# Samirez/Visual_odometry

Measured on AMD Instinct MI355X. Metric: frame-pairs/sec (1280x720, 2000 ORB feats), higher is better.
Workload: dtype u8+f32+f64; 1 GPU; seeded synthetic 1280x720 drone flight (256 distinct rendered views, closed loop), 2000 ORB features/frame, 8 levels = BASELINE config 2; chunk of 257 consecutive frames -> 256 pairs (k, k+1) per GPU per step, each frame detected once; detector=orb, distinct_rendered_frames=256, pair_stride=1, contexts_per_gpu=3, keypoint_order=cv2, poly_solver=fast, matcher=crosscheck, matcher_kernel=mfma_fp4, ransac=5-point, conf 0.99, 1 px, seed 2^64-1, <=1000 iters, parallelism=single GPU, pairs_ok_last_step=256

## Files before the change

### visual_odometry_amd/csrc/cv2order_kernels.hip

```cpp
#include "vo_internal.h"
#include <float.h>

#ifndef CV_THREADS
#define CV_THREADS 256
#endif
#ifndef CV_EPT
#define CV_EPT 4
#endif
#ifndef CV_LDS_CAP
#define CV_LDS_CAP 4096
#endif

__device__ __forceinline__ bool el_gt(uint2 x, uint2 y) { return __uint_as_float(x.x) > __uint_as_float(y.x); }

#define CV_TIE_CAP CV_THREADS
struct Cv2Shared {
    int cnt[2][CV_EPT][CV_THREADS / 64][2];
    int probe[2][CV_THREADS / 64];
    int ntie, nleft;
    uint32_t tie[CV_TIE_CAP], tie_sorted[CV_TIE_CAP], left[CV_TIE_CAP];
    uint8_t is_tie[CV_TIE_CAP];
};

__device__ __forceinline__ void rank2(const bool (&fl)[CV_EPT], const bool (&fr)[CV_EPT], int parity, Cv2Shared& sh,
// ... 265 lines not shown
        for (int j = 0; j < nr; j++) r += sh.tie[j] < p ? 1 : 0;
        sh.tie_sorted[r] = p;
        sh.is_tie[i] = 0;
    }
    __syncthreads();
    for (int i = tid; i < nr; i += CV_THREADS) { const int rel = (int)sh.tie_sorted[i] - first; if (rel < nr) sh.is_tie[rel] = 1; }
    if (tid == 0) sh.nleft = 0;
    __syncthreads();
    {
        const bool fl = tid < nr && first + tid < last && !sh.is_tie[tid];
        const unsigned long long m = __ballot(fl);
        const int lane = tid & 63, wave = tid >> 6;
        if (lane == 0) sh.probe[0][wave] = (int)__popcll(m);
        __syncthreads();
        int before = 0, total = 0;
        for (int w = 0; w < CV_THREADS / 64; w++) { const int c = sh.probe[0][w]; if (w < wave) before += c; total += c; }
        if (fl) sh.left[before + (int)__popcll(m & (lane ? (~0ULL >> (64 - lane)) : 0ULL))] = (uint32_t)(first + tid);
        if (tid == 0) sh.nleft = total;
    }
    __syncthreads();
    const int K = sh.nleft;
    for (int k = tid; k < K; k += CV_THREADS) {
        const int i = (int)sh.left[k], j = (int)sh.tie_sorted[nr - 1 - k];
        const uint2 x = a[i], y = a[j];
        a[i] = y; a[j] = x;
    }
    __syncthreads();
    return first + nr;
}

template <typename PosT>
__device__ int retain_best_cv2(uint2* a, int n, int n_points, PosT* lpos, PosT* rpos, uint2* s_a, uint16_t* s_l, uint16_t* s_r, Cv2Shared& sh)
{
    if (n_points < 0 || n <= n_points) return n;
    if (n_points == 0) return 0;
    const int tid = threadIdx.x;
    int first = 0, last = n;
    const int nth = n_points - 1;
    int depth = 2 * (31 - __clz(n));
    bool done = false;
    introselect_loop(a, first, last, nth, depth, done, CV_LDS_CAP, lpos, rpos, sh);
    if (!done) {
        const int len = last - first;
        for (int i = tid; i < len; i += CV_THREADS) s_a[i] = a[first + i];
        __syncthreads();
        int f2 = 0, l2 = len;
        introselect_loop(s_a, f2, l2, nth - first, depth, done, CV_WAVE_CAP, s_l, s_r, sh);
        if (!done) {
            if (tid < 64) introselect_wave(s_a, f2, l2, nth - first, depth, s_l, s_r);
            __syncthreads();
        }
        for (int i = tid; i < len; i += CV_THREADS) a[first + i] = s_a[i];
        __syncthreads();
    }
    const float ambiguous = __uint_as_float(a[n_points - 1].x);
    const int fast = partition_ge_sparse(a, n_points, n, ambiguous, sh);
    if (fast >= 0) return fast;
    return partition_pass<1>(a, n_points, n, make_uint2(0, 0), ambiguous, lpos, rpos, sh);
}

__global__ __launch_bounds__(CV_THREADS) void k_cv2_order(PyrGeom g, FrameFeat ff, Cv2Buf cb, const int* kept_in)
{
    __shared__ Cv2Shared sh;
    __shared__ uint2 s_a[CV_LDS_CAP];
    __shared__ uint16_t s_l[CV_LDS_CAP], s_r[CV_LDS_CAP];
    const int l = blockIdx.x, f = blockIdx.y, tid = threadIdx.x;
    const LevelGeom lv = g.lv[l];
    const size_t abase = (size_t)f * cb.all_total + cb.all_off[l];
    const uint32_t* all_pos = cb.all_pos + abase;
    const float* all_resp = cb.all_resp + abase;
    uint2* a = cb.work + abase;
    uint32_t* lpos = cb.lpos + abase;
    uint32_t* rpos = cb.rpos + abase;
    const int listed = cb.all_count[f * VO_MAX_LEVELS + l];
    const int n0 = min(listed, cb.all_cap[l]);
    bool bad = listed > cb.all_cap[l];
    for (int i = tid; i < n0; i += CV_THREADS) a[i] = make_uint2(__float_as_uint(all_resp[i]), (uint32_t)i);
    __syncthreads();
    int n = retain_best_cv2(a, n0, g.score_type == 0 ? 2 * lv.quota : lv.quota, lpos, rpos, s_a, s_l, s_r, sh);
    if (g.score_type == 0) {
        const int nc = min(ff.cand_count[f * VO_MAX_LEVELS + l], lv.cand_cap);
        const uint32_t* cpos = ff.cand_pos + (size_t)f * g.cand_total + lv.cand_off;
        const float* cresp = ff.cand_resp + (size_t)f * g.cand_total + lv.cand_off;
        for (int i = tid; i < n; i += CV_THREADS) {
            const uint32_t pos = all_pos[a[i].y];
            int lo = 0, hi = nc;
            while (lo < hi) { const int mid = (lo + hi) >> 1; if (cpos[mid] < pos) lo = mid + 1; else hi = mid; }
            const bool hit = lo < nc && cpos[lo] == pos;
            bad |= !hit;
            a[i].x = __float_as_uint(hit ? cresp[lo] : -FLT_MAX);
        }
        __syncthreads();
        n = retain_best_cv2(a, n, lv.quota, lpos, rpos, s_a, s_l, s_r, sh);
    }
    int out_base = 0;
    for (int k = 0; k < l; k++) out_base += kept_in[f * VO_MAX_LEVELS + k];
    bad |= n != kept_in[f * VO_MAX_LEVELS + l];
    uint32_t* kp_pos = ff.kp_pos + (size_t)f * g.kp_cap;
    int* kp_level = ff.kp_level + (size_t)f * g.kp_cap;
    float* kp_resp = ff.kp_resp + (size_t)f * g.kp_cap;
    const int nw = min(n, kept_in[f * VO_MAX_LEVELS + l]);
    for (int i = tid; i < nw; i += CV_THREADS) {
        const int p = out_base + i;
        if (p < g.kp_cap) { kp_pos[p] = all_pos[a[i].y]; kp_level[p] = l; kp_resp[p] = __uint_as_float(a[i].x); }
    }
    if (bad && tid == 0) atomicOr(&ff.flags[f], 1);
}

void launch_cv2_order(hipStream_t s, const PyrGeom& g, FrameFeat ff, Cv2Buf cb, int F, const int* kept)
{
    hipLaunchKernelGGL(k_cv2_order, dim3(g.nlevels, F), dim3(CV_THREADS), 0, s, g, ff, cb, kept);
}

__global__ __launch_bounds__(CV_THREADS) void k_retain_raw(const float* resp, int n, int n_points, uint2* a, uint32_t* lpos,
                                                          uint32_t* rpos, int* order, int* n_out)
{
    __shared__ Cv2Shared sh;
    __shared__ uint2 s_a[CV_LDS_CAP];
    __shared__ uint16_t s_l[CV_LDS_CAP], s_r[CV_LDS_CAP];
    for (int i = threadIdx.x; i < n; i += CV_THREADS) a[i] = make_uint2(__float_as_uint(resp[i]), (uint32_t)i);
    __syncthreads();
    const int m = retain_best_cv2(a, n, n_points, lpos, rpos, s_a, s_l, s_r, sh);
    for (int i = threadIdx.x; i < m; i += CV_THREADS) order[i] = (int)a[i].y;
    if (threadIdx.x == 0) *n_out = m;
}

void launch_retain_raw(hipStream_t s, const float* resp, int n, int n_points, uint2* a, uint32_t* lpos, uint32_t* rpos,
                       int* order, int* n_out)
{
    hipLaunchKernelGGL(k_retain_raw, dim3(1), dim3(CV_THREADS), 0, s, resp, n, n_points, a, lpos, rpos, order, n_out);
}
```

### visual_odometry_amd/csrc/orb_kernels.hip

```cpp
#include "vo_internal.h"
#include <type_traits>
#include <float.h>
#include <stdlib.h>

__constant__ int8_t c_pattern[256 * 4] = {
#include "orb_pattern.inc"
};
__constant__ int c_umax[16] = {15, 15, 15, 15, 14, 14, 14, 13, 13, 12, 11, 10, 9, 8, 6, 3};
__constant__ int c_gauss7[7] = {18, 34, 49, 55, 49, 34, 18};


typedef short vo_s16x2 __attribute__((ext_vector_type(2)));
typedef unsigned short vo_u16x2 __attribute__((ext_vector_type(2)));
__device__ __forceinline__ uint32_t pk_sub16(uint32_t a, uint32_t b)
{
    return __builtin_bit_cast(uint32_t, __builtin_bit_cast(vo_s16x2, a) - __builtin_bit_cast(vo_s16x2, b));
}
__device__ __forceinline__ uint32_t pk_add16(uint32_t a, uint32_t b)
{
    return __builtin_bit_cast(uint32_t, __builtin_bit_cast(vo_s16x2, a) + __builtin_bit_cast(vo_s16x2, b));
}
__device__ __forceinline__ uint32_t pk_min16(uint32_t a, uint32_t b)
{
    return __builtin_bit_cast(uint32_t, __builtin_elementwise_min(__builtin_bit_cast(vo_s16x2, a), __builtin_bit_cast(vo_s16x2, b)));
// ... 636 lines not shown
            __syncthreads();
            for (int e0 = 0, k = 0; e0 < nc; e0 += 64, k++)
                if ((lose >> k) & 1u) { const int q = s_q[e0 + lane]; s_sc[(q >> 8) * FT_SCW + (q & 255)] = 0; }
            __syncthreads();
        }
    } else {
        for (int i = lane; i < FT_SCH * (FAST_TW + 2); i += 64) {
            const int gr = i / (FAST_TW + 2), cx = 3 + i % (FAST_TW + 2);
            const int gx = x0 - 4 + cx, gy = y0 - 1 + gr;
            if (gx < xlo || gx > xhi || gy < gylo || gy > gyhi) continue;
            s_sc[gr * FT_SCW + cx] = (uint8_t)fast_score_or_zero(s_px + (gr + 3) * FT_PXW + 12 + cx, t);
        }
        __syncthreads();
        uint8_t* s_out = s_px;
        for (int i = lane; i < FAST_TH * FAST_TW; i += 64) {
            const int ty = i / FAST_TW, tx = i % FAST_TW;
            const uint8_t* c = s_sc + (ty + 1) * FT_SCW + 4 + tx;
            const int sv = c[0];
            const bool win = sv && sv > c[-1] && sv > c[1] && sv > c[-FT_SCW - 1] && sv > c[-FT_SCW] && sv > c[-FT_SCW + 1] &&
                             sv > c[FT_SCW - 1] && sv > c[FT_SCW] && sv > c[FT_SCW + 1];
            s_out[i] = win ? (uint8_t)sv : 0;
            const int gx = x0 + tx, gy = y0 + ty;
            const bool keep = win && gx >= g.edge && gx < lv.w - g.edge && gy >= g.edge && gy < lv.h - g.edge;
            if (keep) atomicAdd(&hist[((size_t)f * VO_MAX_LEVELS + l) * 256 + sv], 1u);
            if (!DENSE) {
                const unsigned long long m = __ballot(keep);
                const int slot = nw + (int)__builtin_amdgcn_mbcnt_hi((uint32_t)(m >> 32), __builtin_amdgcn_mbcnt_lo((uint32_t)m, 0u));
                if (keep) my_list[slot] = ((uint32_t)sv << 16) | ((uint32_t)ty << 8) | (uint32_t)tx;
                nw += (int)__popcll(m);
            }
        }
        __syncthreads();
        for (int i = lane; i < FAST_TH * FAST_TW; i += 64) s_sc[(i / FAST_TW + 1) * FT_SCW + 4 + i % FAST_TW] = s_out[i];
        __syncthreads();
    }
    if (!DENSE) {
        FT_STAT(4, nw);
        if (lane == 0) tile_count[(size_t)f * g.ftiles_total + bid] = nw;
        return;
    }
#pragma unroll
    for (int i = lane; i < FAST_TH * (FAST_TW / 16); i += 64) {
        const int ty = i / (FAST_TW / 16), c16 = i % (FAST_TW / 16);
        const int gy = y0 + ty, gx = x0 + 16 * c16;
        const uint32_t* c = (const uint32_t*)(s_sc + (ty + 1) * FT_SCW + 4 + 16 * c16);
        if (gy < lv.h && gx < lv.stride)
            *(uint4*)(score + (size_t)f * g.frame_bytes + lv.off + (size_t)gy * lv.stride + gx) = make_uint4(c[0], c[1], c[2], c[3]);
    }
}

static_assert((FAST_TH * FAST_TW) % 64 == 0, "the dense fallback appends with full-wave ballots");
void launch_fast(hipStream_t s, const uint8_t* pyr, uint8_t* score, uint32_t* hist, const PyrGeom& g, int F,
                 uint32_t* tile_list, int* tile_count)
{
    if (tile_list) { if (g.ftiles_total > 0) hipLaunchKernelGGL(k_fast<false>, dim3(g.ftiles_total, F), dim3(64), 0, s, pyr, score, hist, g, tile_list, tile_count); }
    else hipLaunchKernelGGL(k_fast<true>, dim3(g.dtiles_total, F), dim3(64), 0, s, pyr, score, hist, g, tile_list, tile_count);
}


__device__ __forceinline__ int sel_threshold(const PyrGeom& g, const LevelGeom& lv, const uint32_t* h, int lane)
{
    const int want = g.score_type == 0 ? 2 * lv.quota : lv.quota;
    uint32_t c[4];
    int own = 0;
#pragma unroll
    for (int k = 0; k < 4; k++) { c[k] = h[255 - 4 * lane - k]; own += (int)c[k]; }
    int inc = own;
#pragma unroll
    for (int d = 1; d < 64; d <<= 1) { int v = __shfl_up(inc, d, 64); if (lane >= d) inc += v; }
    int acc = inc - own, T = 0;
#pragma unroll
    for (int k = 0; k < 4; k++) {
        acc += (int)c[k];
        const int score = 255 - 4 * lane - k;
        if (T == 0 && acc >= want && score >= 1) T = score;
    }
    const unsigned long long found = __ballot(T != 0);
    int result = 1;
    if (found) result = __shfl(T, __ffsll((long long)found) - 1, 64);
    if (want <= 0 || lv.w <= 2 * g.edge || lv.h <= 2 * g.edge) result = 256;
    return __builtin_amdgcn_readfirstlane(result);
}

template <bool EMIT, bool ALL>
__device__ __forceinline__ void sel_rows(const uint32_t* tile_list, const int* tile_count, const PyrGeom& g, const FrameFeat& ff,
                                         int* thr, int* chunk_count, const Cv2Buf& cb, uint32_t* s_sel)
{
    const int f = blockIdx.y, lane = threadIdx.x;
    int l = 0;
    while (l + 1 < g.nlevels && (int)blockIdx.x >= g.lv[l + 1].sel_chunk_base) l++;
    const LevelGeom lv = g.lv[l];
    const int chunk = blockIdx.x - lv.sel_chunk_base;
    const int nchunks = (l + 1 < g.nlevels ? g.lv[l + 1].sel_chunk_base : g.sel_chunks_total) - lv.sel_chunk_base;
    const size_t cslot = (size_t)f * g.sel_chunks_total + blockIdx.x;
    const size_t tile0 = (size_t)f * g.ftiles_total + lv.ftile_base + (size_t)chunk * lv.ftiles_x;
    if (!EMIT) {
        const int T = sel_threshold(g, lv, ff.hist + ((size_t)f * VO_MAX_LEVELS + l) * 256, lane);
        int n = 0, na = 0;
        if (ALL || T <= 255)
            for (int t = 0; t < lv.ftiles_x; t++) {
                const int cnt = min(tile_count[tile0 + t], FT_LISTCAP);
                const uint32_t* lst = tile_list + (tile0 + t) * FT_LISTCAP;
                na += cnt;
                for (int j0 = 0; j0 < cnt; j0 += 64) {
                    const int j = j0 + lane;
                    const uint32_t e = j < cnt ? lst[j] : 0u;
                    n += (int)__popcll(__ballot(j < cnt && (int)(e >> 16) >= T));
                }
            }
        if (lane != 0) return;
        chunk_count[cslot] = n;
        if (ALL) cb.chunk_count[cslot] = na;
        if (chunk == 0) thr[f * VO_MAX_LEVELS + l] = T;
        if (blockIdx.x == 0) {
            ff.flags[f] = 0;
            for (int k = 0; k < g.nlevels; k++)
                if ((k + 1 < g.nlevels ? g.lv[k + 1].sel_chunk_base : g.sel_chunks_total) == g.lv[k].sel_chunk_base) {
                    ff.cand_count[f * VO_MAX_LEVELS + k] = 0;
                    if (ALL) cb.all_count[f * VO_MAX_LEVELS + k] = 0;
                }
        }
        return;
    }
    const int T = thr[f * VO_MAX_LEVELS + l];
    if (!ALL && T > 255) {
        if (chunk == 0 && lane == 0) ff.cand_count[f * VO_MAX_LEVELS + l] = 0;
        return;
    }
    int base = 0, abase = 0;
    {
        const size_t c0 = (size_t)f * g.sel_chunks_total + lv.sel_chunk_base;
        for (int c = lane; c < chunk; c += 64) { base += chunk_count[c0 + c]; if (ALL) abase += cb.chunk_count[c0 + c]; }
#pragma unroll
        for (int d = 32; d >= 1; d >>= 1) { base += __shfl_xor(base, d, 64); if (ALL) abase += __shfl_xor(abase, d, 64); }
    }
    const int W32 = (lv.w + 31) >> 5, NW = FAST_TH * W32;
    uint32_t* s_bm = s_sel;
    uint32_t* s_pf = s_sel + NW;
    uint32_t* s_abm = s_sel + 2 * NW;
    uint32_t* s_apf = s_sel + 3 * NW;
    for (int i = lane; i < NW; i += 64) { s_bm[i] = 0u; if (ALL) s_abm[i] = 0u; }
    __syncthreads();
    for (int t = 0; t < lv.ftiles_x; t++) {
        const int cnt = min(tile_count[tile0 + t], FT_LISTCAP);
        const uint32_t* lst = tile_list + (tile0 + t) * FT_LISTCAP;
        for (int j = lane; j < cnt; j += 64) {
            const uint32_t e = lst[j];
            const bool kept = (int)(e >> 16) >= T;
            if (ALL || kept) {
                const uint32_t gx = (uint32_t)(lv.fox + t * FAST_TW) + (e & 255u), wd = ((e >> 8) & 255u) * W32 + (gx >> 5), bit = 1u << (gx & 31u);
                if (ALL) atomicOr(&s_abm[wd], bit);
                if (kept) atomicOr(&s_bm[wd], bit);
            }
        }
    }
    __syncthreads();
    int n, na = 0;
    {
        const int per = (NW + 63) / 64, w0 = lane * per, w1 = min(NW, w0 + per);
        int own = 0, aown = 0;
        for (int wd = w0; wd < w1; wd++) { own += __popc(s_bm[wd]); if (ALL) aown += __popc(s_abm[wd]); }
        int inc = own, ainc = aown;
#pragma unroll
        for (int d = 1; d < 64; d <<= 1) {
            const int v = __shfl_up(inc, d, 64); if (lane >= d) inc += v;
            if (ALL) { const int av = __shfl_up(ainc, d, 64); if (lane >= d) ainc += av; }
        }
        n = __shfl(inc, 63, 64);
        if (ALL) na = __shfl(ainc, 63, 64);
        int acc = inc - own, aacc = ainc - aown;
        for (int wd = w0; wd < w1; wd++) {
            s_pf[wd] = (uint32_t)acc; acc += __popc(s_bm[wd]);
            if (ALL) { s_apf[wd] = (uint32_t)aacc; aacc += __popc(s_abm[wd]); }
        }
    }
    __syncthreads();
    bool overflow = false;
    uint32_t* out_pos = ff.cand_pos + (size_t)f * g.cand_total + lv.cand_off;
    float* out_resp = ff.cand_resp + (size_t)f * g.cand_total + lv.cand_off;
    uint32_t* all_pos = ALL ? cb.all_pos + (size_t)f * cb.all_total + cb.all_off[l] : nullptr;
    float* all_resp = ALL ? cb.all_resp + (size_t)f * cb.all_total + cb.all_off[l] : nullptr;
    const int all_cap = ALL ? cb.all_cap[l] : 0;
    for (int t = 0; t < lv.ftiles_x; t++) {
        const int cnt = min(tile_count[tile0 + t], FT_LISTCAP);
        const uint32_t* lst = tile_list + (tile0 + t) * FT_LISTCAP;
        for (int j = lane; j < cnt; j += 64) {
            const uint32_t e = lst[j];
            const bool kept = (int)(e >> 16) >= T;
            if (ALL || kept) {
                const uint32_t ly = (e >> 8) & 255u, gx = (uint32_t)(lv.fox + t * FAST_TW) + (e & 255u);
                const int wd = (int)(ly * W32 + (gx >> 5));
                const uint32_t below = (1u << (gx & 31u)) - 1u, key = (((uint32_t)(lv.foy + chunk * FAST_TH) + ly) << 16) | gx;
                const float score = (float)(e >> 16);
                if (ALL) {
                    const int apos = abase + (int)s_apf[wd] + __popc(s_abm[wd] & below);
                    if (apos < all_cap) { all_pos[apos] = key; all_resp[apos] = score; }
                    else overflow = true;
                }
                if (kept) {
                    const int pos = base + (int)s_pf[wd] + __popc(s_bm[wd] & below);
                    if (pos < lv.cand_cap) { out_pos[pos] = key; out_resp[pos] = score; }
                    else overflow = true;
                }
            }
        }
    }
    if (overflow) atomicOr(&ff.flags[f], 1);
    if (chunk == nchunks - 1 && lane == 0) {
        ff.cand_count[f * VO_MAX_LEVELS + l] = min(base + n, lv.cand_cap);
        if (ALL) cb.all_count[f * VO_MAX_LEVELS + l] = min(abase + na, all_cap);
    }
}

template <bool EMIT>
__global__ __launch_bounds__(64) void k_sel_rows(const uint32_t* tile_list, const int* tile_count, PyrGeom g, FrameFeat ff,
                                                 int* thr, int* chunk_count)
{
    extern __shared__ uint32_t s_sel[];
    sel_rows<EMIT, false>(tile_list, tile_count, g, ff, thr, chunk_count, Cv2Buf(), s_sel);
}
template <bool EMIT>
__global__ __launch_bounds__(64) void k_sel_rows(const uint32_t* tile_list, const int* tile_count, PyrGeom g, FrameFeat ff,
                                                 int* thr, int* chunk_count, Cv2Buf cb)
{
    extern __shared__ uint32_t s_sel[];
    sel_rows<EMIT, true>(tile_list, tile_count, g, ff, thr, chunk_count, cb, s_sel);
}

static size_t sel_bitmap_bytes(const PyrGeom& g, bool all)
{
    int w = 0;
    for (int l = 0; l < g.nlevels; l++) w = g.lv[l].w > w ? g.lv[l].w : w;
    return (size_t)(all ? 4 : 2) * FAST_TH * ((w + 31) / 32) * 4;
}

void launch_select_fast(hipStream_t s, const PyrGeom& g, FrameFeat ff, int F, int* thr, int* chunk_count,
                        const uint32_t* tile_list, const int* tile_count, const Cv2Buf* cb)
{
    if (g.sel_chunks_total <= 0) {
        (void)hipMemsetAsync(ff.flags, 0, (size_t)F * sizeof(int), s);
        (void)hipMemsetAsync(ff.cand_count, 0, (size_t)F * VO_MAX_LEVELS * sizeof(int), s);
        if (cb) (void)hipMemsetAsync(cb->all_count, 0, (size_t)F * VO_MAX_LEVELS * sizeof(int), s);
        return;
    }
    const dim3 grid(g.sel_chunks_total, F);
    if (cb) {
        hipLaunchKernelGGL(k_sel_rows<false>, grid, dim3(64), 0, s, tile_list, tile_count, g, ff, thr, chunk_count, *cb);
        hipLaunchKernelGGL(k_sel_rows<true>, grid, dim3(64), sel_bitmap_bytes(g, true), s, tile_list, tile_count, g, ff, thr, chunk_count, *cb);
    } else {
        hipLaunchKernelGGL(k_sel_rows<false>, grid, dim3(64), 0, s, tile_list, tile_count, g, ff, thr, chunk_count);
        hipLaunchKernelGGL(k_sel_rows<true>, grid, dim3(64), sel_bitmap_bytes(g, false), s, tile_list, tile_count, g, ff, thr, chunk_count);
    }
}

__global__ __launch_bounds__(256) void k_harris(const uint8_t* pyr, PyrGeom g, FrameFeat ff, int blocks_per_level)
{
    const int bid = xcd_tile(blockIdx.x, gridDim.x);
    const int f = bid / (blocks_per_level * g.nlevels), l = (bid / blocks_per_level) % g.nlevels;
    const int i = (bid % blocks_per_level) * 256 + threadIdx.x;
    const LevelGeom lv = g.lv[l];
    if (i >= min(ff.cand_count[f * VO_MAX_LEVELS + l], lv.cand_cap)) return;
    const size_t ci = (size_t)f * g.cand_total + lv.cand_off + i;
    const uint32_t pos = ff.cand_pos[ci];
    const int x0 = pos & 0xffff, y0 = pos >> 16, st = lv.stride;
    const uint8_t* img = pyr + (size_t)f * g.frame_bytes + lv.off + (size_t)(y0 - 4) * st + (x0 - 4);
    int dxr[9][7], sxr[9][7];
#pragma unroll
    for (int r = 0; r < 9; r++) {
        uint32_t w0, w1, w2;
        __builtin_memcpy(&w0, img + (size_t)r * st, 4);
        __builtin_memcpy(&w1, img + (size_t)r * st + 4, 4);
        __builtin_memcpy(&w2, img + (size_t)r * st + 8, 4);
        int px[9];
#pragma unroll
        for (int c = 0; c < 9; c++) px[c] = (int)(((c < 4 ? w0 : c < 8 ? w1 : w2) >> (8 * (c & 3))) & 255u);
#pragma unroll
        for (int c = 0; c < 7; c++) { dxr[r][c] = px[c + 2] - px[c]; sxr[r][c] = px[c] + 2 * px[c + 1] + px[c + 2]; }
    }
    int a = 0, b = 0, c = 0;
#pragma unroll
    for (int r = 1; r < 8; r++)
#pragma unroll
        for (int k = 0; k < 7; k++) {
            const int Ix = dxr[r - 1][k] + 2 * dxr[r][k] + dxr[r + 1][k];
            const int Iy = sxr[r + 1][k] - sxr[r - 1][k];
            a += Ix * Ix; b += Iy * Iy; c += Ix * Iy;
        }
    const float scale = 1.f / ((1 << 2) * 7 * 255.f);
    const float scale_sq_sq = scale * scale * scale * scale;
    ff.cand_resp[ci] = ((float)a * (float)b - (float)c * (float)c - 0.04f * ((float)a + (float)b) * ((float)a + (float)b)) * scale_sq_sq;
}

void launch_harris(hipStream_t s, const uint8_t* pyr, const PyrGeom& g, FrameFeat ff, int F)
{
    int maxcap = 0;
    for (int l = 0; l < g.nlevels; l++) maxcap = g.lv[l].cand_cap > maxcap ? g.lv[l].cand_cap : maxcap;
    const int bpl = (maxcap + 255) / 256;
    hipLaunchKernelGGL(k_harris, dim3(bpl * g.nlevels * F), dim3(256), 0, s, pyr, g, ff, bpl);
}

__device__ __forceinline__ uint32_t f2key(float v)
{
    uint32_t u = __float_as_uint(v);
    return (u & 0x80000000u) ? ~u : (u | 0x80000000u);
}
__device__ __forceinline__ float key2f(uint32_t k)
{
    return __uint_as_float((k & 0x80000000u) ? (k & 0x7fffffffu) : ~k);
}

__global__ __launch_bounds__(256) void k_harris_threshold(PyrGeom g, FrameFeat ff, float* thr_out, int* kept_out)
{
    __shared__ int s_hist[256];
    __shared__ uint32_t s_prefix;
    __shared__ int s_remaining;
    __shared__ int s_kept;
// ... 563 lines not shown
```

### visual_odometry_amd/csrc/vo_api.hip

```cpp
#include "vo_internal.h"
#include <float.h>
#include <math.h>
#include <stdio.h>
#include <stdlib.h>
#include <string.h>
#include <vector>
#include <type_traits>
#include <algorithm>

#define MAX_EVENTS 384

struct DevList {
    struct Entry { void* p; bool pinned; };
    std::vector<Entry> ptrs;
    DevList() = default;
    DevList(const DevList&) = delete;
    DevList& operator=(DevList&& o) noexcept { if (this != &o) { release(); ptrs.swap(o.ptrs); } return *this; }
    ~DevList() { release(); }
    template <typename T> hipError_t alloc(T** p, size_t n) { return keep(hipMalloc((void**)p, (n ? n : 1) * sizeof(T)), (void**)p, false); }
    template <typename T> hipError_t alloc_pinned(T** p, size_t n)
    {
        return keep(hipHostMalloc((void**)p, (n ? n : 1) * sizeof(T), hipHostMallocDefault), (void**)p, true);
    }
    void release()
// ... 233 lines not shown
        const int iw = lv.w - p->edge_threshold - lv.fox, ih = lv.h - p->edge_threshold - lv.foy;
        const int trows = iw > 0 && ih > 0 ? (ih + FAST_TH - 1) / FAST_TH : 0;
        lv.ftile_base = ft; lv.ftiles_x = trows > 0 ? (iw + FAST_TW - 1) / FAST_TW : 0;
        ft += lv.ftiles_x * trows;
        lv.dtile_base = dt; lv.dtiles_x = (lv.w + FAST_TW - 1) / FAST_TW;
        dt += lv.dtiles_x * ((lv.h + FAST_TH - 1) / FAST_TH);
        lv.btile_base = bt; lv.btiles_x = (lv.w + BLUR_TW - 1) / BLUR_TW;
        bt += lv.btiles_x * ((lv.h + BLUR_TH - 1) / BLUR_TH);
        const int want = p->score_type == 0 ? 2 * lv.quota : lv.quota;
        lv.sel_chunk_base = sc;
        sc += trows;
        lv.cand_off = co;
        lv.cand_cap = align_up(want + (want > 1024 ? want : 1024), 8);
        co += lv.cand_cap;
    }
    g->frame_bytes = align_up(off, 256);
    g->ftiles_total = ft; g->btiles_total = bt; g->dtiles_total = dt;
    g->cand_total = co;
    g->sel_chunks_total = sc;
    g->kp_cap = align_up(p->nfeatures + (p->nfeatures / 8 > 256 ? p->nfeatures / 8 : 256), 8);
    return VO_OK;
}

static void build_lin_tab(int ssize, int dsize, int* ofs, uint16_t* c1, int* pmin, int* pmax)
{
    const double inv_scale = (double)dsize / (double)ssize;
    const double scale = 1.0 / inv_scale;
    int minofst = 0, maxofst = dsize;
    for (int val = 0; val < dsize; val++) {
        volatile double fval = scale * ((double)val + 0.5);
        fval = fval - 0.5;
        const double fv = fval;
        const int ival = cv_floor_d(fv);
        ofs[val] = 0; c1[val] = 0;
        if (ival >= 0 && ssize > 1) {
            if (ival < ssize - 1) {
                ofs[val] = ival;
                volatile double fr = fv - (double)ival;
                fr = fr * 256.0;
                c1[val] = (uint16_t)lrint((double)fr);
            } else {
                ofs[val] = ssize - 1;
                if (val < maxofst) maxofst = val;
            }
        } else if (val + 1 > minofst) minofst = val + 1;
    }
    *pmin = minofst; *pmax = maxofst;
}

static hipError_t alloc_pairbuf(DevList& mem, PairBuf& pb, int P, int cap, bool with_pose_mask)
{
    hipError_t e;
    const size_t pc = (size_t)P * cap;
    pb = PairBuf{};
#define A_(field, n) if ((e = mem.alloc(&pb.field, (n))) != hipSuccess) return e
    A_(slots, (size_t)P * 2); A_(nn_idx, pc * 2); A_(nn_dist, pc * 2); A_(nn_idx2, pc); A_(nn_dist2, pc);
    A_(m_q, pc); A_(m_t, pc); A_(m_d, pc); A_(m_count, (size_t)P);
    A_(px1, pc * 2); A_(px2, pc * 2); A_(xn1, pc * 2); A_(xn2, pc * 2);
    A_(mask, pc); A_(models, (size_t)P * 64 * 90); A_(pose_state, (size_t)P);
    A_(in1, pc * 2); A_(in2, pc * 2); A_(ipx1, pc * 2); A_(ipx2, pc * 2);
    A_(res, (size_t)P); A_(X, pc * 4);
    if (with_pose_mask) { A_(pose_mask, pc); }
    if (const size_t n = nn_colkey_ints(P, cap)) { A_(nn_colkey, n); }
#undef A_
    return hipSuccess;
}

static int alloc_cv2(vo_ctx* ctx)
{
    if (ctx->cv2_ready) return VO_OK;
    const PyrGeom& g = ctx->g;
    Cv2Buf& cb = ctx->cv2;
    int off = 0;
    for (int l = 0; l < g.nlevels; l++) {
        const int px8 = g.lv[l].w * g.lv[l].h / 8 + 1024;
        cb.all_off[l] = off;
        cb.all_cap[l] = align_up(px8 > g.lv[l].cand_cap ? px8 : g.lv[l].cand_cap, 8);
        off += cb.all_cap[l];
    }
    cb.all_total = off;
    const size_t F = (size_t)ctx->max_frames, n = F * off;
    DevList& m = ctx->orb_mem;
    HIPCHK(m.alloc(&cb.all_pos, n)); HIPCHK(m.alloc(&cb.all_resp, n)); HIPCHK(m.alloc(&cb.work, n));
    HIPCHK(m.alloc(&cb.lpos, n)); HIPCHK(m.alloc(&cb.rpos, n));
    HIPCHK(m.alloc(&cb.all_count, F * VO_MAX_LEVELS));
    HIPCHK(m.alloc(&cb.chunk_count, F * (size_t)(g.sel_chunks_total + 1)));
    HIPCHK(hipMemset(cb.all_count, 0, F * VO_MAX_LEVELS * sizeof(int)));
    HIPCHK(hipDeviceSynchronize());
    ctx->cv2_ready = true;
    return VO_OK;
}

static void free_config(vo_ctx* c)
{
    c->configured = c->cv2_ready = false;
    c->orb_mem.release();
    c->pb_mem.release();
    c->pb_pairs = c->pb_cap = 0;
    clear_last_run(c);
}

static void comm_release(vo_ctx* ctx);
static int sift_frames_upload_enqueue(vo_ctx* ctx, const uint8_t* frames, int F, int row_stride, int64_t frame_stride, int first_slot);
static int sift_frames_detect_enqueue(vo_ctx* ctx, int first_slot, int F);

extern "C" int vo_version(void) { return 120; }

extern "C" int vo_create(int device_id, vo_ctx** out)
{
    if (!out) return VO_ERR_INVALID;
    *out = nullptr;
    int ndev = 0;
    if (hipGetDeviceCount(&ndev) != hipSuccess || device_id < 0 || device_id >= ndev) return VO_ERR_HIP;
    vo_ctx* ctx = new vo_ctx();
    ctx->device = device_id;
    if (hipSetDevice(device_id) != hipSuccess || hipStreamCreateWithFlags(&ctx->stream, hipStreamNonBlocking) != hipSuccess ||
        ctx->mem.alloc(&ctx->dK, 16) != hipSuccess) {
        delete ctx;
        return VO_ERR_HIP;
    }
    for (int i = 0; i < MAX_EVENTS; i++) { (void)hipEventCreate(&ctx->ev[i][0]); (void)hipEventCreate(&ctx->ev[i][1]); }
    ctx->ev_ready = true;
    (void)hipEventCreateWithFlags(&ctx->ev_det, hipEventDisableTiming);
    *out = ctx;
    return VO_OK;
}

extern "C" void vo_destroy(vo_ctx* ctx)
{
    if (!ctx) return;
    (void)hipSetDevice(ctx->device);
    (void)hipStreamSynchronize(ctx->stream);
    if (ctx->stream_jpg) { (void)hipStreamSynchronize(ctx->stream_jpg); (void)hipStreamDestroy(ctx->stream_jpg); }
    for (int i = 0; i < 2; i++) if (ctx->ev_jpg[i]) (void)hipEventDestroy(ctx->ev_jpg[i]);
    if (ctx->ev_ready) for (int i = 0; i < MAX_EVENTS; i++) { (void)hipEventDestroy(ctx->ev[i][0]); (void)hipEventDestroy(ctx->ev[i][1]); }
    if (ctx->ev_det) (void)hipEventDestroy(ctx->ev_det);
    comm_release(ctx);
    (void)hipStreamDestroy(ctx->stream);
    delete ctx;
}

enum { NN_POPCOUNT, NN_INT8, NN_FP4 };
static int nn_kernel(const vo_ctx* ctx, int cap)
{
    if (ctx->matcher_kernel == 1 || cap >= 16129) return NN_POPCOUNT;
    return ctx->matcher_kernel == 2 && cap < 8192 ? NN_FP4 : NN_INT8;
}

static int launch_hamming_nn(const vo_ctx* ctx, const PairBuf& pb, const uint8_t* desc, const uint8_t* desc_x, int fp4,
                             const int* kp_count, int cap, int P, int dirs, int knn2)
{
    if (nn_kernel(ctx, cap) == NN_POPCOUNT) { launch_match_nn_popcount(ctx->stream, desc, kp_count, cap, pb, P, dirs, knn2); return 0; }
    return launch_match_nn(ctx->stream, desc_x, kp_count, cap, desc_x_rows(cap), pb, P, dirs, knn2, fp4);
}

extern "C" int vo_set_matcher_kernel(vo_ctx* ctx, int kind)
{
    if (!ctx) return VO_ERR_INVALID;
    if (kind < 0 || kind > 2) FAIL(VO_ERR_INVALID, "matcher kernel must be 0 (int8 MFMA), 1 (XOR + popcount) or 2 (block-scaled FP4 MFMA)");
    ctx->matcher_kernel = kind;
    return VO_OK;
}

extern "C" int vo_set_keypoint_order(vo_ctx* ctx, int kind)
{
    if (!ctx) return VO_ERR_INVALID;
    if (kind != 0 && kind != 1) FAIL(VO_ERR_INVALID, "keypoint order must be 0 (canonical) or 1 (cv2)");
// ... 155 lines not shown
    if (row_stride == ctx->w && frame_stride >= (int64_t)ctx->w * ctx->h) {
        const size_t per = (size_t)ctx->w * ctx->h;
        int rc = ctx->staging.grow(ctx, per * F); if (rc) return rc;
        HIPCHK(hipMemcpy2DAsync(ctx->staging.p, per, frames, (size_t)frame_stride, per, F, hipMemcpyHostToDevice, ctx->stream));
        launch_gray(ctx->stream, ctx->staging.p, 1, ctx->w, (int64_t)per, ctx->pyr + (size_t)first_slot * ctx->g.frame_bytes, ctx->g, F);
        HIPCHK(hipGetLastError());
        return VO_OK;
    }
    for (int f = 0; f < F; f++)
        HIPCHK(hipMemcpy2DAsync(dst0 + (size_t)f * ctx->g.frame_bytes, lv.stride, frames + (size_t)f * frame_stride, row_stride,
                                ctx->w, ctx->h, hipMemcpyHostToDevice, ctx->stream));
    return VO_OK;
}

extern "C" int vo_frames_upload(vo_ctx* ctx, const uint8_t* frames, int F, int row_stride, int64_t frame_stride, int first_slot)
{
    if (!ctx) return VO_ERR_INVALID;
    int rc = frames_upload_enqueue(ctx, frames, F, row_stride, frame_stride, first_slot);
    if (rc) return rc;
    HIPCHK(hipStreamSynchronize(ctx->stream));
    return VO_OK;
}

extern "C" int vo_frames_upload_async(vo_ctx* ctx, const uint8_t* frames, int F, int row_stride, int64_t frame_stride, int first_slot)
{
    if (!ctx) return VO_ERR_INVALID;
    return frames_upload_enqueue(ctx, frames, F, row_stride, frame_stride, first_slot);
}

extern "C" int vo_frames_upload_color(vo_ctx* ctx, const uint8_t* frames, int F, int channels, int row_stride,
                                      int64_t frame_stride, int first_slot)
{
    if (!ctx) return VO_ERR_INVALID;
    if (channels == 1) return vo_frames_upload(ctx, frames, F, row_stride, frame_stride, first_slot);
    const Batch b = batch(ctx);
    if (!b.ready) FAIL(VO_ERR_NOT_CONFIGURED, "vo_batch_configure has not been called");
    if (channels != 3 && channels != 4) FAIL(VO_ERR_INVALID, "channels must be 1, 3 or 4");
    if (!frames || F < 0 || first_slot < 0 || first_slot + F > b.max_frames) FAIL(VO_ERR_INVALID, "slot range out of bounds");
    if (row_stride < b.w * channels || frame_stride < (int64_t)row_stride * b.h) FAIL(VO_ERR_INVALID, "strides too small");
    if (F == 0) return VO_OK;
    HIPCHK(hipSetDevice(ctx->device));
    const size_t per = (size_t)frame_stride;
    const int chunk = F < 64 ? F : 64;
    int rc = ctx->staging.grow(ctx, per * chunk); if (rc) return rc;
    for (int f0 = 0; f0 < F; f0 += chunk) {
        const int n = F - f0 < chunk ? F - f0 : chunk;
        HIPCHK(hipMemcpyAsync(ctx->staging.p, frames + (size_t)f0 * per, per * n, hipMemcpyHostToDevice, ctx->stream));
        StageTimer t(ctx, ST_GRAY);
        gray_into_slots(ctx, ctx->stream, ctx->staging.p, channels, row_stride, frame_stride, first_slot + f0, n);
    }
    HIPCHK(hipGetLastError());
    HIPCHK(hipStreamSynchronize(ctx->stream));
    if (ctx->prof) prof_collect(ctx);
    return VO_OK;
}

static int run_detect(vo_ctx* ctx, int first_slot, int F, int upto)
{
    const PyrGeom& g = ctx->g;
    hipStream_t s = ctx->stream;
    uint8_t* pyr = ctx->pyr + (size_t)first_slot * g.frame_bytes;
    uint8_t* blur = ctx->blur + (size_t)first_slot * g.frame_bytes;
    uint8_t* score = ctx->score + (size_t)first_slot * g.frame_bytes;
    FrameFeat ff = ctx->ff;
    ff.cand_pos += (size_t)first_slot * g.cand_total; ff.cand_resp += (size_t)first_slot * g.cand_total;
    ff.cand_count += (size_t)first_slot * VO_MAX_LEVELS;
    ff.kp_pos += (size_t)first_slot * g.kp_cap; ff.kp_level += (size_t)first_slot * g.kp_cap;
    ff.kp_resp += (size_t)first_slot * g.kp_cap; ff.kp_angle += (size_t)first_slot * g.kp_cap;
    ff.kp_xy += (size_t)first_slot * g.kp_cap * 2; ff.kp_size += (size_t)first_slot * g.kp_cap;
    ff.desc += (size_t)first_slot * g.kp_cap * 32;
    ff.kp_count += first_slot; ff.flags += first_slot;
    ff.hist += (size_t)first_slot * VO_MAX_LEVELS * 256;
    ff.tile_list += (size_t)first_slot * g.ftiles_total * FAST_LISTCAP; ff.tile_count += (size_t)first_slot * g.ftiles_total;
    {
        StageTimer t(ctx, ST_RESIZE);
        for (int l = 1; l < g.nlevels; l++) launch_resize(s, pyr, g, l, ctx->tabs[l], F);
    }
    if (upto < 1) return VO_OK;
    const bool cv2 = ctx->kp_order == 1 && ctx->cv2_ready;
    Cv2Buf cb = ctx->cv2;
    if (cv2) {
        const size_t fo = (size_t)first_slot;
        cb.all_pos += fo * cb.all_total; cb.all_resp += fo * cb.all_total; cb.work += fo * cb.all_total;
        cb.lpos += fo * cb.all_total; cb.rpos += fo * cb.all_total;
        cb.all_count += fo * VO_MAX_LEVELS; cb.chunk_count += fo * g.sel_chunks_total;
    }
    {
        StageTimer t(ctx, ST_MISC);
        HIPCHK(hipMemsetAsync(ff.hist, 0, (size_t)F * VO_MAX_LEVELS * 256 * sizeof(uint32_t), s));
        if (upto < 2) {
            HIPCHK(hipMemsetAsync(ff.flags, 0, (size_t)F * sizeof(int), s));
            HIPCHK(hipMemsetAsync(ff.cand_count, 0, (size_t)F * VO_MAX_LEVELS * sizeof(int), s));
            if (cv2) HIPCHK(hipMemsetAsync(cb.all_count, 0, (size_t)F * VO_MAX_LEVELS * sizeof(int), s));
        }
    }
    { StageTimer t(ctx, ST_FAST); launch_fast(s, pyr, score, ff.hist, g, F, upto < 2 ? nullptr : ff.tile_list, ff.tile_count); }
    if (upto < 2) return VO_OK;
    { StageTimer t(ctx, ST_SELECT_FAST); launch_select_fast(s, g, ff, F, ctx->sel_thr + (size_t)first_slot * VO_MAX_LEVELS, ctx->sel_chunk_count + (size_t)first_slot * g.sel_chunks_total, ff.tile_list, ff.tile_count, cv2 ? &cb : nullptr); }
    if (g.score_type == 0) { StageTimer t(ctx, ST_HARRIS); launch_harris(s, pyr, g, ff, F); }
    { StageTimer t(ctx, ST_SELECT_HARRIS); launch_select_harris(s, g, ff, F, ctx->har_thr + (size_t)first_slot * VO_MAX_LEVELS, ctx->har_kept + (size_t)first_slot * VO_MAX_LEVELS); }
    if (cv2) {
        StageTimer t(ctx, ST_CV2_ORDER);
        launch_cv2_order(s, g, ff, cb, F, ctx->har_kept + (size_t)first_slot * VO_MAX_LEVELS);
    }
    { StageTimer t(ctx, ST_ANGLE); launch_angle(s, pyr, g, ff, F); }
    { StageTimer t(ctx, ST_BLUR); launch_blur(s, pyr, blur, g, F); }
    {
        StageTimer t(ctx, ST_BRIEF);
        const int cx = desc_x_rows(g.kp_cap);
        ctx->descx_fp4 = nn_kernel(ctx, g.kp_cap) == NN_FP4;
        launch_brief(s, blur, g, ff, F, ctx->desc_x + (size_t)first_slot * cx * 256, cx, ctx->descx_fp4);
    }
    return VO_OK;
}

extern "C" int vo_batch_kp_capacity(vo_ctx* ctx)
{
    if (!ctx) return 0;
    const Batch b = batch(ctx);
    return b.ready ? b.kp_cap : 0;
}

extern "C" int vo_host_alloc(size_t bytes, void** out)
{
    if (!out) return VO_ERR_INVALID;
    *out = nullptr;
    return hipHostMalloc(out, bytes ? bytes : 1, hipHostMallocDefault) == hipSuccess ? VO_OK : VO_ERR_HIP;
}

extern "C" void vo_host_free(void* p)
{
    if (p) (void)hipHostFree(p);
}

static int detect_enqueue(vo_ctx* ctx, int first_slot, int F)
{
    const Batch b = batch(ctx);
    if (!b.ready) FAIL(VO_ERR_NOT_CONFIGURED, "vo_batch_configure has not been called");
    if (F < 0 || first_slot < 0 || first_slot + F > b.max_frames) FAIL(VO_ERR_INVALID, "slot range out of bounds");
    HIPCHK(hipSetDevice(ctx->device));
    if (F == 0) return VO_OK;
    if (b.sift) return sift_frames_detect_enqueue(ctx, first_slot, F);
    int rc = run_detect(ctx, first_slot, F, 2);
    if (rc) return rc;
    HIPCHK(hipGetLastError());
    return VO_OK;
}

extern "C" int vo_frames_detect_async(vo_ctx* ctx, int first_slot, int F)
{
    if (!ctx) return VO_ERR_INVALID;
    int rc = detect_enqueue(ctx, first_slot, F);
    if (rc) return rc;
    HIPCHK(hipEventRecord(ctx->ev_det, ctx->stream));
    ctx->ev_det_set = true;
    return VO_OK;
}

extern "C" int vo_detect_after(vo_ctx* ctx, vo_ctx* other)
{
    if (!ctx || !other) return VO_ERR_INVALID;
    if (ctx->device != other->device) FAIL(VO_ERR_INVALID, "the two contexts are on different devices");
    if (ctx == other || !other->ev_det_set) return VO_OK;
    HIPCHK(hipSetDevice(ctx->device));
    HIPCHK(hipStreamWaitEvent(ctx->stream, other->ev_det, 0));
    return VO_OK;
}
// ... 2275 lines not shown
```

### visual_odometry_amd/csrc/vo_internal.h

```cpp
#pragma once
#include <hip/hip_runtime.h>
#include <stdint.h>
#include "../../include/vo_hip.h"

enum {
    ST_GRAY = 0, ST_RESIZE, ST_FAST, ST_SELECT_FAST, ST_HARRIS, ST_SELECT_HARRIS, ST_ANGLE,
    ST_BLUR, ST_BRIEF, ST_MATCH_NN, ST_MATCH_SELECT, ST_RANSAC, ST_POSE, ST_TRIANGULATE,
    ST_MISC, ST_RESERVED, ST_SIFT_SCALE, ST_SIFT_EXTREMA, ST_SIFT_ORIENT, ST_SIFT_SORT, ST_SIFT_DESC, ST_CV2_ORDER, ST_GATHER, ST_RESERVED2,
    ST_SLAM_PREPARE, ST_SLAM_BA, ST_SLAM_FILTER, ST_SLAM_LIMIT
};

struct LevelGeom {
    int w, h, stride, off;
    int quota;
    float scale;
    int ftile_base, ftiles_x;
    int fox, foy;
    int dtile_base, dtiles_x;
    int btile_base, btiles_x;
    int cand_off, cand_cap;
    int sel_chunk_base;
};

struct PyrGeom {
    int nlevels, frame_bytes;
    int edge, fast_thr, score_type, nfeatures;
    int ftiles_total, btiles_total, dtiles_total;
    int cand_total, kp_cap;
    int sel_chunks_total;
    LevelGeom lv[VO_MAX_LEVELS];
};

#define RS2_WW 256
#define RS2_WH 16
#ifndef RS2_WAVES
#define RS2_WAVES 4
#endif
#define RS2_THREADS (64 * RS2_WAVES)
#define RS2_TH (RS2_WAVES * RS2_WH)

struct ResizeTab {
    const int* xofs; const uint16_t* xc1;
    const int* yofs; const uint16_t* yc1;
    int min_x, max_x, min_y, max_y;
    int direct;
};

#ifndef FAST_TW
#define FAST_TW 112
#endif
#ifndef FAST_TH
#define FAST_TH 20
#endif
#define BLUR_TW 128
#ifndef BLUR_TH
#define BLUR_TH 48
#endif
#define FAST_LISTCAP ((FAST_TW / 2) * (FAST_TH / 2))

struct FrameFeat {
    uint32_t* cand_pos;
    float*    cand_resp;
    int*      cand_count;
    uint32_t* kp_pos;
    int*      kp_level;
    float*    kp_resp;
    float*    kp_angle;
    float*    kp_xy;
    float*    kp_size;
    uint8_t*  desc;
    int*      kp_count;
    int*      flags;
    uint32_t* hist;
    uint32_t* tile_list;
    int*      tile_count;
};

struct Cv2Buf {
    uint32_t* all_pos;
    float*    all_resp;
    int*      all_count;
    int*      chunk_count;
    uint2*    work;
    uint32_t* lpos;
    uint32_t* rpos;
    int all_off[VO_MAX_LEVELS], all_cap[VO_MAX_LEVELS], all_total;
};

struct PoseState {
    int active;
    int ninl;
    int good[4];
    double R1[9], R2[9], t[3];
};

struct PairBuf {
    int*      slots;
    int*      nn_idx;
    int*      nn_dist;
    int*      nn_idx2;
    int*      nn_dist2;
    int*      nn_colkey;
    int*      m_q;
    int*      m_t;
    float*    m_d;
    int*      m_count;
    double*   px1;
    double*   px2;
    double*   xn1;
    double*   xn2;
    uint8_t*  mask;
    double*   models;
    PoseState* pose_state;
    double*   in1;
    double*   in2;
    double*   ipx1;
    double*   ipx2;
    vo_pair_result* res;
    double*   X;
    uint8_t*  pose_mask;
};

struct RansacParams {
    double prob, thresh_px;
    int max_iters;
    uint64_t seed;
    double K[9];
    double dist_thresh;
    int dk_early;
};

const char* rccl_load(void);
const char* rccl_unique_id(uint8_t* id128);
const char* rccl_comm_init(void** comm, const uint8_t* id128, int rank, int world);
void rccl_comm_destroy(void* comm);
const char* rccl_comm_count(void* comm, int* n);
const char* rccl_all_gather_f64(void* comm, const double* send, double* recv, size_t count, hipStream_t s);
void launch_pack_records(hipStream_t s, const vo_pair_result* res, int B, int valid, double* rec);

void launch_gray(hipStream_t s, const uint8_t* src, int channels, int row_stride, int64_t frame_stride,
                 uint8_t* pyr, const PyrGeom& g, int F);
void launch_gray_plain(hipStream_t s, const uint8_t* src, int channels, int row_stride, int64_t frame_stride,
                       uint8_t* dst, int w, int h, int dstride, int64_t dframe, int F);
void launch_resize(hipStream_t s, uint8_t* pyr, const PyrGeom& g, int level, const ResizeTab& tab, int F);
void launch_fast(hipStream_t s, const uint8_t* pyr, uint8_t* score, uint32_t* hist, const PyrGeom& g, int F,
                 uint32_t* tile_list, int* tile_count);
void launch_select_fast(hipStream_t s, const PyrGeom& g, FrameFeat ff, int F, int* thr, int* chunk_count,
                        const uint32_t* tile_list, const int* tile_count, const Cv2Buf* cb);
void launch_harris(hipStream_t s, const uint8_t* pyr, const PyrGeom& g, FrameFeat ff, int F);
void launch_cv2_order(hipStream_t s, const PyrGeom& g, FrameFeat ff, Cv2Buf cb, int F, const int* kept);
void launch_retain_raw(hipStream_t s, const float* resp, int n, int n_points, uint2* a, uint32_t* lpos, uint32_t* rpos,
                       int* order, int* n_out);
void launch_select_harris(hipStream_t s, const PyrGeom& g, FrameFeat ff, int F, float* thr, int* kept);
void launch_angle(hipStream_t s, const uint8_t* pyr, const PyrGeom& g, FrameFeat ff, int F);
void launch_resize_linear(hipStream_t st, const uint8_t* src, int sw, int sh, int cn, int sstride, int64_t sframe,
                          uint8_t* dst, int dw, int dh, int dstride, int64_t dframe,
                          const int* xofs, const void* xa, const int* yofs, const void* yb, int area2, int F);
void launch_resize_area(hipStream_t st, const uint8_t* src, int cn, int sstride, uint8_t* dst, int dw, int dh, int dstride,
                        int isx, int isy, const int* xsi, const float* xal, const int* xst, const int* ysi, const float* yal, const int* yst);
#define SIFT_IMG_BORDER 5
#define SIFT_MAX_INTERP_STEPS 5
#define SIFT_MAX_OCT 16
#define SIFT_MAX_TAPS 64
// ... 156 lines not shown
```

Baseline: 98370 frame-pairs/s.

## Flatten FAST tile-list traversal and record candidate indices to skip binary search

The select-FAST kernel now walks the per-tile lists through a wave-wide prefix scan over tile counts, so each lane processes several flattened entries per trip instead of looping tile by tile with mostly idle lanes. The first batch of entries is packed and held in registers across the marking and emit passes. During emit it records each kept entry's candidate index into a new all_cand buffer, which lets the cv2-order kernel replace its per-element binary search over candidate positions with a direct indexed lookup. The prefix arrays can optionally be 16-bit to shrink LDS use. In exchange it adds an extra global buffer and write, more register pressure, and readlane loops over up to 64 tiles per entry batch.

New measurement: 101,000 frame-pairs/s, median of 6. +2.7%, better.

```diff
diff --git a/visual_odometry_amd/csrc/cv2order_kernels.hip b/visual_odometry_amd/csrc/cv2order_kernels.hip
--- a/visual_odometry_amd/csrc/cv2order_kernels.hip
+++ b/visual_odometry_amd/csrc/cv2order_kernels.hip
@@ -371,13 +371,12 @@
         const int nc = min(ff.cand_count[f * VO_MAX_LEVELS + l], lv.cand_cap);
         const uint32_t* cpos = ff.cand_pos + (size_t)f * g.cand_total + lv.cand_off;
         const float* cresp = ff.cand_resp + (size_t)f * g.cand_total + lv.cand_off;
+        const uint32_t* all_cand = cb.all_cand + abase;
         for (int i = tid; i < n; i += CV_THREADS) {
-            const uint32_t pos = all_pos[a[i].y];
-            int lo = 0, hi = nc;
-            while (lo < hi) { const int mid = (lo + hi) >> 1; if (cpos[mid] < pos) lo = mid + 1; else hi = mid; }
-            const bool hit = lo < nc && cpos[lo] == pos;
+            const uint32_t ai = a[i].y, pos = all_pos[ai], idx = all_cand[ai];
+            const bool hit = idx < (uint32_t)nc && cpos[idx] == pos;
             bad |= !hit;
-            a[i].x = __float_as_uint(hit ? cresp[lo] : -FLT_MAX);
+            a[i].x = __float_as_uint(hit ? cresp[idx] : -FLT_MAX);
         }
         __syncthreads();
         n = retain_best_cv2(a, n, lv.quota, lpos, rpos, s_a, s_l, s_r, sh);
diff --git a/visual_odometry_amd/csrc/orb_kernels.hip b/visual_odometry_amd/csrc/orb_kernels.hip
--- a/visual_odometry_amd/csrc/orb_kernels.hip
+++ b/visual_odometry_amd/csrc/orb_kernels.hip
@@ -742,6 +742,43 @@
     return __builtin_amdgcn_readfirstlane(result);
 }
 
+__device__ __forceinline__ int sel_load_counts(const int* tile_count, size_t tile_first, int nt, int lane)
+{
+    return min(tile_count[tile_first + min(lane, max(nt - 1, 0))], FT_LISTCAP);
+}
+__device__ __forceinline__ int sel_scan_counts(int cnt, int nt, int lane, int& total)
+{
+    int inc = cnt;
+#pragma unroll
+    for (int d = 1; d < 64; d <<= 1) { const int v = __shfl_up(inc, d, 64); if (lane >= d) inc += v; }
+    total = __builtin_amdgcn_readlane(inc, max(nt - 1, 0));
+    return inc;
+}
+
+#define SEL_TRIPS 4
+__device__ __forceinline__ void sel_flat_entries(const uint32_t* lists, int nt, int inc, int e, int total,
+                                                 uint32_t (&ent)[SEL_TRIPS], int (&tile)[SEL_TRIPS])
+{
+    int st[SEL_TRIPS];
+#pragma unroll
+    for (int u = 0; u < SEL_TRIPS; u++) { tile[u] = 0; st[u] = 0; }
+    for (int k = 0; k + 1 < nt; k++) {
+        const int v = __builtin_amdgcn_readlane(inc, k);
+#pragma unroll
+        for (int u = 0; u < SEL_TRIPS; u++) if (e + 64 * u >= v) { tile[u] = k + 1; st[u] = v; }
+    }
+#pragma unroll
+    for (int u = 0; u < SEL_TRIPS; u++) ent[u] = lists[e + 64 * u < total ? tile[u] * FT_LISTCAP + (e + 64 * u - st[u]) : 0];
+#pragma unroll
+    for (int u = 0; u < SEL_TRIPS; u++) ent[u] = e + 64 * u < total ? ent[u] : 0u;
+}
+
+#ifdef SEL_PF16
+typedef uint16_t sel_pf_t;
+#else
+typedef uint32_t sel_pf_t;
+#endif
+
 template <bool EMIT, bool ALL>
 __device__ __forceinline__ void sel_rows(const uint32_t* tile_list, const int* tile_count, const PyrGeom& g, const FrameFeat& ff,
                                          int* thr, int* chunk_count, const Cv2Buf& cb, uint32_t* s_sel)
@@ -755,17 +792,22 @@
     const size_t cslot = (size_t)f * g.sel_chunks_total + blockIdx.x;
     const size_t tile0 = (size_t)f * g.ftiles_total + lv.ftile_base + (size_t)chunk * lv.ftiles_x;
     if (!EMIT) {
+        int cnt = sel_load_counts(tile_count, tile0, min(lv.ftiles_x, 64), lane);
         const int T = sel_threshold(g, lv, ff.hist + ((size_t)f * VO_MAX_LEVELS + l) * 256, lane);
         int n = 0, na = 0;
         if (ALL || T <= 255)
-            for (int t = 0; t < lv.ftiles_x; t++) {
-                const int cnt = min(tile_count[tile0 + t], FT_LISTCAP);
-                const uint32_t* lst = tile_list + (tile0 + t) * FT_LISTCAP;
-                na += cnt;
-                for (int j0 = 0; j0 < cnt; j0 += 64) {
-                    const int j = j0 + lane;
-                    const uint32_t e = j < cnt ? lst[j] : 0u;
-                    n += (int)__popcll(__ballot(j < cnt && (int)(e >> 16) >= T));
+            for (int tb = 0; tb < lv.ftiles_x; tb += 64) {
+                const int nt = min(lv.ftiles_x - tb, 64);
+                if (tb) cnt = sel_load_counts(tile_count, tile0 + tb, nt, lane);
+                int total;
+                const int inc = sel_scan_counts(cnt, nt, lane, total);
+                const uint32_t* lists = tile_list + (tile0 + tb) * FT_LISTCAP;
+                na += total;
+                for (int e0 = 0; e0 < total; e0 += 64 * SEL_TRIPS) {
+                    uint32_t ent[SEL_TRIPS]; int tile[SEL_TRIPS];
+                    sel_flat_entries(lists, nt, inc, e0 + lane, total, ent, tile);
+#pragma unroll
+                    for (int u = 0; u < SEL_TRIPS; u++) n += (int)__popcll(__ballot((int)(ent[u] >> 16) >= T));
                 }
             }
         if (lane != 0) return;
@@ -782,6 +824,8 @@
         }
         return;
     }
+    const int nt0 = min(lv.ftiles_x, 64);
+    const int cnt0 = sel_load_counts(tile_count, tile0, nt0, lane);
     const int T = thr[f * VO_MAX_LEVELS + l];
     if (!ALL && T > 255) {
         if (chunk == 0 && lane == 0) ff.cand_count[f * VO_MAX_LEVELS + l] = 0;
@@ -794,26 +838,49 @@
 #pragma unroll
         for (int d = 32; d >= 1; d >>= 1) { base += __shfl_xor(base, d, 64); if (ALL) abase += __shfl_xor(abase, d, 64); }
     }
+    auto pack = [&](uint32_t e, int tile) -> uint32_t {
+        return e ? ((e & 0x00ff0000u) << 8) | ((e & 0x0000ff00u) << 8) | ((uint32_t)(lv.fox + tile * FAST_TW) + (e & 255u)) : 0u;
+    };
+    int total0;
+    const int inc0 = sel_scan_counts(cnt0, nt0, lane, total0);
+    uint32_t held[SEL_TRIPS];
+    {
+        uint32_t ent[SEL_TRIPS]; int tile[SEL_TRIPS];
+        sel_flat_entries(tile_list + tile0 * FT_LISTCAP, nt0, inc0, lane, total0, ent, tile);
+#pragma unroll
+        for (int u = 0; u < SEL_TRIPS; u++) held[u] = pack(ent[u], tile[u]);
+    }
+    auto beyond_held = [&](auto&& visit) {
+        for (int tb = 0; tb < lv.ftiles_x; tb += 64) {
+            const int nt = min(lv.ftiles_x - tb, 64);
+            int total = total0, inc = inc0;
+            if (tb) inc = sel_scan_counts(sel_load_counts(tile_count, tile0 + tb, nt, lane), nt, lane, total);
+            for (int e0 = tb ? 0 : 64 * SEL_TRIPS; e0 < total; e0 += 64 * SEL_TRIPS) {
+                uint32_t ent[SEL_TRIPS]; int tile[SEL_TRIPS];
+                sel_flat_entries(tile_list + (tile0 + tb) * FT_LISTCAP, nt, inc, e0 + lane, total, ent, tile);
+#pragma unroll
+                for (int u = 0; u < SEL_TRIPS; u++) visit(pack(ent[u], tb + tile[u]));
+            }
+        }
+    };
     const int W32 = (lv.w + 31) >> 5, NW = FAST_TH * W32;
     uint32_t* s_bm = s_sel;
-    uint32_t* s_pf = s_sel + NW;
-    uint32_t* s_abm = s_sel + 2 * NW;
-    uint32_t* s_apf = s_sel + 3 * NW;
+    uint32_t* s_abm = s_sel + NW;
+    sel_pf_t* s_pf = (sel_pf_t*)(s_sel + (ALL ? 2 : 1) * NW);
+    sel_pf_t* s_apf = s_pf + NW;
     for (int i = lane; i < NW; i += 64) { s_bm[i] = 0u; if (ALL) s_abm[i] = 0u; }
     __syncthreads();
-    for (int t = 0; t < lv.ftiles_x; t++) {
-        const int cnt = min(tile_count[tile0 + t], FT_LISTCAP);
-        const uint32_t* lst = tile_list + (tile0 + t) * FT_LISTCAP;
-        for (int j = lane; j < cnt; j += 64) {
-            const uint32_t e = lst[j];
-            const bool kept = (int)(e >> 16) >= T;
-            if (ALL || kept) {
-                const uint32_t gx = (uint32_t)(lv.fox + t * FAST_TW) + (e & 255u), wd = ((e >> 8) & 255u) * W32 + (gx >> 5), bit = 1u << (gx & 31u);
-                if (ALL) atomicOr(&s_abm[wd], bit);
-                if (kept) atomicOr(&s_bm[wd], bit);
-            }
-        }
-    }
+    auto mark = [&](uint32_t p) {
+        const bool kept = (int)(p >> 24) >= T;
+        if (ALL ? p != 0u : kept) {
+            const uint32_t gx = p & 0xffffu, wd = ((p >> 16) & 255u) * W32 + (gx >> 5), bit = 1u << (gx & 31u);
+            if (ALL) atomicOr(&s_abm[wd], bit);
+            if (kept) atomicOr(&s_bm[wd], bit);
+        }
+    };
+#pragma unroll
+    for (int u = 0; u < SEL_TRIPS; u++) mark(held[u]);
+    beyond_held(mark);
     __syncthreads();
     int n, na = 0;
     {
@@ -830,8 +897,8 @@
         if (ALL) na = __shfl(ainc, 63, 64);
         int acc = inc - own, aacc = ainc - aown;
         for (int wd = w0; wd < w1; wd++) {
-            s_pf[wd] = (uint32_t)acc; acc += __popc(s_bm[wd]);
-            if (ALL) { s_apf[wd] = (uint32_t)aacc; aacc += __popc(s_abm[wd]); }
+            s_pf[wd] = (sel_pf_t)acc; acc += __popc(s_bm[wd]);
+            if (ALL) { s_apf[wd] = (sel_pf_t)aacc; aacc += __popc(s_abm[wd]); }
         }
     }
     __syncthreads();
@@ -840,31 +907,34 @@
     float* out_resp = ff.cand_resp + (size_t)f * g.cand_total + lv.cand_off;
     uint32_t* all_pos = ALL ? cb.all_pos + (size_t)f * cb.all_total + cb.all_off[l] : nullptr;
     float* all_resp = ALL ? cb.all_resp + (size_t)f * cb.all_total + cb.all_off[l] : nullptr;
+    uint32_t* all_cand = ALL ? cb.all_cand + (size_t)f * cb.all_total + cb.all_off[l] : nullptr;
     const int all_cap = ALL ? cb.all_cap[l] : 0;
-    for (int t = 0; t < lv.ftiles_x; t++) {
-        const int cnt = min(tile_count[tile0 + t], FT_LISTCAP);
-        const uint32_t* lst = tile_list + (tile0 + t) * FT_LISTCAP;
-        for (int j = lane; j < cnt; j += 64) {
-            const uint32_t e = lst[j];
-            const bool kept = (int)(e >> 16) >= T;
-            if (ALL || kept) {
-                const uint32_t ly = (e >> 8) & 255u, gx = (uint32_t)(lv.fox + t * FAST_TW) + (e & 255u);
-                const int wd = (int)(ly * W32 + (gx >> 5));
-                const uint32_t below = (1u << (gx & 31u)) - 1u, key = (((uint32_t)(lv.foy + chunk * FAST_TH) + ly) << 16) | gx;
-                const float score = (float)(e >> 16);
-                if (ALL) {
-                    const int apos = abase + (int)s_apf[wd] + __popc(s_abm[wd] & below);
-                    if (apos < all_cap) { all_pos[apos] = key; all_resp[apos] = score; }
-                    else overflow = true;
+    auto emit = [&](uint32_t p) {
+        const bool kept = (int)(p >> 24) >= T;
+        if (ALL ? p != 0u : kept) {
+            const uint32_t ly = (p >> 16) & 255u, gx = p & 0xffffu;
+            const int wd = (int)(ly * W32 + (gx >> 5));
+            const uint32_t below = (1u << (gx & 31u)) - 1u, key = (((uint32_t)(lv.foy + chunk * FAST_TH) + ly) << 16) | gx;
+            const float score = (float)(p >> 24);
+            int pos = 0;
+            if (kept) {
+                pos = base + (int)s_pf[wd] + __popc(s_bm[wd] & below);
+                if (pos < lv.cand_cap) { out_pos[pos] = key; out_resp[pos] = score; }
+                else overflow = true;
+            }
+            if (ALL) {
+                const int apos = abase + (int)s_apf[wd] + __popc(s_abm[wd] & below);
+                if (apos < all_cap) {
+                    all_pos[apos] = key; all_resp[apos] = score;
+                    if (kept) all_cand[apos] = (uint32_t)pos;
                 }
-                if (kept) {
-                    const int pos = base + (int)s_pf[wd] + __popc(s_bm[wd] & below);
-                    if (pos < lv.cand_cap) { out_pos[pos] = key; out_resp[pos] = score; }
-                    else overflow = true;
-                }
+                else overflow = true;
             }
         }
-    }
+    };
+#pragma unroll
+    for (int u = 0; u < SEL_TRIPS; u++) emit(held[u]);
+    beyond_held(emit);
     if (overflow) atomicOr(&ff.flags[f], 1);
     if (chunk == nchunks - 1 && lane == 0) {
         ff.cand_count[f * VO_MAX_LEVELS + l] = min(base + n, lv.cand_cap);
@@ -891,7 +961,7 @@
 {
     int w = 0;
     for (int l = 0; l < g.nlevels; l++) w = g.lv[l].w > w ? g.lv[l].w : w;
-    return (size_t)(all ? 4 : 2) * FAST_TH * ((w + 31) / 32) * 4;
+    return (size_t)(all ? 2 : 1) * FAST_TH * ((w + 31) / 32) * (sizeof(uint32_t) + sizeof(sel_pf_t));
 }
 
 void launch_select_fast(hipStream_t s, const PyrGeom& g, FrameFeat ff, int F, int* thr, int* chunk_count,
diff --git a/visual_odometry_amd/csrc/vo_api.hip b/visual_odometry_amd/csrc/vo_api.hip
--- a/visual_odometry_amd/csrc/vo_api.hip
+++ b/visual_odometry_amd/csrc/vo_api.hip
@@ -339,7 +339,7 @@
     const size_t F = (size_t)ctx->max_frames, n = F * off;
     DevList& m = ctx->orb_mem;
     HIPCHK(m.alloc(&cb.all_pos, n)); HIPCHK(m.alloc(&cb.all_resp, n)); HIPCHK(m.alloc(&cb.work, n));
-    HIPCHK(m.alloc(&cb.lpos, n)); HIPCHK(m.alloc(&cb.rpos, n));
+    HIPCHK(m.alloc(&cb.all_cand, n)); HIPCHK(m.alloc(&cb.lpos, n)); HIPCHK(m.alloc(&cb.rpos, n));
     HIPCHK(m.alloc(&cb.all_count, F * VO_MAX_LEVELS));
     HIPCHK(m.alloc(&cb.chunk_count, F * (size_t)(g.sel_chunks_total + 1)));
     HIPCHK(hipMemset(cb.all_count, 0, F * VO_MAX_LEVELS * sizeof(int)));
@@ -661,7 +661,7 @@
     if (cv2) {
         const size_t fo = (size_t)first_slot;
         cb.all_pos += fo * cb.all_total; cb.all_resp += fo * cb.all_total; cb.work += fo * cb.all_total;
-        cb.lpos += fo * cb.all_total; cb.rpos += fo * cb.all_total;
+        cb.all_cand += fo * cb.all_total; cb.lpos += fo * cb.all_total; cb.rpos += fo * cb.all_total;
         cb.all_count += fo * VO_MAX_LEVELS; cb.chunk_count += fo * g.sel_chunks_total;
     }
     {
diff --git a/visual_odometry_amd/csrc/vo_internal.h b/visual_odometry_amd/csrc/vo_internal.h
--- a/visual_odometry_amd/csrc/vo_internal.h
+++ b/visual_odometry_amd/csrc/vo_internal.h
@@ -79,6 +79,7 @@
 struct Cv2Buf {
     uint32_t* all_pos;
     float*    all_resp;
+    uint32_t* all_cand;
     int*      all_count;
     int*      chunk_count;
     uint2*    work;
```
